# mttga/purejaxql

Hardware: NVIDIA H100
Metric: MinAtar-Breakout env steps/sec @4096 envs x128 seeds (higher is better)
Workload: dtype f32

## Files before the change

### purejaxql_b200/csrc/conv16.cuh

```cuda
#pragma once
#include <cuda_fp16.h>
#include <cuda_runtime.h>
#include <stdint.h>

#include "../../include/pqn_b200.h"
#include "tc_common.cuh"

namespace pqn {

constexpr float LN_EPS = 1e-6f;
constexpr int CONV_O = 16;
constexpr int CONV_PIX = 64;
constexpr int HID_CNN = 128;
constexpr int FLAT_CNN = CONV_PIX * CONV_O;

template <int C>
struct ConvCfg {
  static constexpr int TAPS = 9 * C;
  static constexpr int OBS_BITS = 100 * C;
  static constexpr int OBS_WORDS = (OBS_BITS + 31) / 32;
  static constexpr int PW = (OBS_WORDS + 3) / 4 * 4;
  static constexpr int SW = PW + 1;
};

template <int C>
struct PatchCfg {
  static constexpr int WORDS = (9 * C + 31) / 32;
};

template <int C>
__device__ __forceinline__ void patch_bits(const uint32_t* __restrict__ so, int pix, uint32_t (&w)[PatchCfg<C>::WORDS]) {
  constexpr int W = PatchCfg<C>::WORDS;
#pragma unroll
  for (int k = 0; k < W; ++k) w[k] = 0u;
  const int y = pix >> 3, x = pix & 7;
#pragma unroll
  for (int di = 0; di < 3; ++di) {
    const int f0 = ((y + di) * 10 + x) * C;
    const uint32_t r = __funnelshift_r(so[f0 >> 5], so[(f0 >> 5) + 1], f0 & 31) & ((1u << (3 * C)) - 1u);
    const int o = 3 * C * di;
    w[o >> 5] |= r << (o & 31);
    if ((o & 31) + 3 * C > 32) w[min((o >> 5) + 1, W - 1)] |= r >> (32 - (o & 31));
  }
}

__device__ __forceinline__ void ln16_quad(const float (&z)[2][4], float& mean0, float& rstd0, float& mean1,
                                          float& rstd1) {
  float s0 = z[0][0] + z[0][1] + z[1][0] + z[1][1];
  float q0 = fmaf(z[1][1], z[1][1], fmaf(z[1][0], z[1][0], fmaf(z[0][0], z[0][0], __fmul_rn(z[0][1], z[0][1]))));
  float s1 = z[0][2] + z[0][3] + z[1][2] + z[1][3];
  float q1 = fmaf(z[1][3], z[1][3], fmaf(z[1][2], z[1][2], fmaf(z[0][2], z[0][2], __fmul_rn(z[0][3], z[0][3]))));
#pragma unroll
  for (int o = 1; o <= 2; o <<= 1) {
    s0 += __shfl_xor_sync(0xffffffffu, s0, o); q0 += __shfl_xor_sync(0xffffffffu, q0, o);
    s1 += __shfl_xor_sync(0xffffffffu, s1, o); q1 += __shfl_xor_sync(0xffffffffu, q1, o);
  }
  mean0 = __fmul_rn(s0, 1.0f / CONV_O); mean1 = __fmul_rn(s1, 1.0f / CONV_O);
  rstd0 = rsqrtf(fmaxf(fmaf(q0, 1.0f / CONV_O, -__fmul_rn(mean0, mean0)), 0.f) + LN_EPS);
  rstd1 = rsqrtf(fmaxf(fmaf(q1, 1.0f / CONV_O, -__fmul_rn(mean1, mean1)), 0.f) + LN_EPS);
}

__device__ __forceinline__ void mma_f16_16n8k16(float (&d)[4], const uint32_t (&a)[4], uint32_t b0, uint32_t b1) {
  asm volatile(
      "mma.sync.aligned.m16n8k16.row.col.f32.f16.f16.f32 {%0,%1,%2,%3}, {%4,%5,%6,%7}, {%8,%9}, {%0,%1,%2,%3};"
      : "+f"(d[0]), "+f"(d[1]), "+f"(d[2]), "+f"(d[3])
      : "r"(a[0]), "r"(a[1]), "r"(a[2]), "r"(a[3]), "r"(b0), "r"(b1));
}

template <int C>
struct Conv16 {
  static constexpr int TAPS = 9 * C;
  static constexpr int KS = (TAPS + 15) / 16;
  static constexpr int ROW = 2 * KS < 8 ? 8 : 2 * KS;
};

__host__ __device__ constexpr int conv16_channel(int h, int n) { return 4 * (n >> 1) + 2 * h + (n & 1); }

__host__ __device__ constexpr int conv16_tap(int s, int kk) {
  return 16 * s + (kk < 8 ? 0 : 8) + ((kk & 1) ? 4 : 0) + ((kk & 7) >> 1);
}

template <int C>
__device__ __forceinline__ void conv16_load_weights(const float* __restrict__ prm, const pqn_net_layout_t& L, uint4* wb,
                                                    float* cb, float* sc, float* bi, int tid, int nt) {
  using M = Conv16<C>;
  const float inv255 = 1.0f / 255.0f;
  for (int i = tid; i < M::KS * 2 * 32; i += nt) {
    const int ln = i & 31, h = (i >> 5) & 1, s = i >> 6;
    const int gg = ln >> 2, tt = ln & 3;
    const int o = conv16_channel(h, gg);
    const float scale = __uint_as_float((uint32_t)(127 + 15 - (1 << tt)) << 23);
    float v[4];
#pragma unroll
    for (int q = 0; q < 4; ++q) {
      const int tap = conv16_tap(s, 2 * tt + (q & 1) + (q >> 1) * 8);
      v[q] = tap < M::TAPS ? __ldg(prm + L.conv_w + tap * CONV_O + o) * inv255 * scale : 0.f;
      v[q] = fminf(fmaxf(v[q], -65000.f), 65000.f);
    }
    const __half2 h0 = __floats2half2_rn(v[0], v[1]), h1 = __floats2half2_rn(v[2], v[3]);
    const float2 f0 = __half22float2(h0), f1 = __half22float2(h1);
    const __half2 l0 = __floats2half2_rn(v[0] - f0.x, v[1] - f0.y), l1 = __floats2half2_rn(v[2] - f1.x, v[3] - f1.y);
    wb[i] = make_uint4(*reinterpret_cast<const uint32_t*>(&h0), *reinterpret_cast<const uint32_t*>(&h1),
                       *reinterpret_cast<const uint32_t*>(&l0), *reinterpret_cast<const uint32_t*>(&l1));
  }
  if (tid < CONV_O) {
    cb[tid] = __ldg(prm + L.conv_b + tid);
    sc[tid] = __ldg(prm + L.ln0_scale + tid);
    bi[tid] = __ldg(prm + L.ln0_bias + tid);
  }
}

template <int C>
__device__ __forceinline__ void build_patch16(const uint32_t* __restrict__ so, int pix, uint32_t* __restrict__ out) {
  constexpr int W = PatchCfg<C>::WORDS;
  uint32_t w[W];
  patch_bits<C>(so, pix, w);
#pragma unroll
  for (int b = 0; b < 2 * Conv16<C>::KS; ++b) {
    const int o = 8 * b;
    uint32_t v = (o >> 5) < W ? w[(o >> 5) < W ? (o >> 5) : 0] : 0u;
    const int sh = o & 31;
    const uint32_t lo = sh >= 10 ? v >> (sh - 10) : v << (10 - sh);
    const uint32_t hi = sh + 4 <= 26 ? v << (26 - sh - 4) : v >> (sh + 4 - 26);
    out[b] = __byte_perm(lo, hi, 0x7610);
  }
}

template <int C>
__device__ __forceinline__ void store_patch16(const uint32_t* __restrict__ so, int pix, uint32_t* __restrict__ row) {
  using M = Conv16<C>;
  uint32_t w[M::ROW];
#pragma unroll
  for (int k = 0; k < M::ROW; ++k) w[k] = 0u;
  build_patch16<C>(so, pix, w);
#pragma unroll
  for (int q = 0; q < M::ROW / 4; ++q)
    *reinterpret_cast<uint4*>(row + 4 * q) = make_uint4(w[4 * q], w[4 * q + 1], w[4 * q + 2], w[4 * q + 3]);
}

template <int C, int NB>
__device__ __forceinline__ void conv16_blocks(const uint32_t* __restrict__ xp, const uint4* __restrict__ wb,
                                              const float* __restrict__ cb, int mb0, int lane, float (&z)[NB][2][4]) {
  using M = Conv16<C>;
  const int g = lane >> 2, t = lane & 3;
  const uint32_t mask = (1u << (10 + t)) | (1u << (26 + t));
#pragma unroll
  for (int i = 0; i < NB; ++i)
#pragma unroll
    for (int h = 0; h < 2; ++h) {
      z[i][h][0] = z[i][h][2] = cb[4 * t + 2 * h];
      z[i][h][1] = z[i][h][3] = cb[4 * t + 2 * h + 1];
    }
  const uint32_t* r00 = xp + (16 * mb0 + g) * M::ROW;
#pragma unroll
  for (int s = 0; s < M::KS; ++s) {
    uint32_t a[NB][4];
#pragma unroll
    for (int i = 0; i < NB; ++i) {
      const uint2 w0 = *reinterpret_cast<const uint2*>(r00 + (16 * i) * M::ROW + 2 * s);
      const uint2 w1 = *reinterpret_cast<const uint2*>(r00 + (16 * i + 8) * M::ROW + 2 * s);
      a[i][0] = w0.x & mask; a[i][1] = w1.x & mask; a[i][2] = w0.y & mask; a[i][3] = w1.y & mask;
    }
    uint4 b[2];
#pragma unroll
    for (int h = 0; h < 2; ++h) b[h] = wb[(s * 2 + h) * 32 + lane];
#pragma unroll
    for (int h = 0; h < 2; ++h)
#pragma unroll
      for (int i = 0; i < NB; ++i) mma_f16_16n8k16(z[i][h], a[i], b[h].z, b[h].w);
#pragma unroll
    for (int h = 0; h < 2; ++h)
#pragma unroll
      for (int i = 0; i < NB; ++i) mma_f16_16n8k16(z[i][h], a[i], b[h].x, b[h].y);
  }
}

__device__ __forceinline__ void conv16_xhat(const float (&z)[2][4], float (&x0)[4], float (&x1)[4], float& rstd0,
                                            float& rstd1) {
  float mean0, mean1;
  ln16_quad(z, mean0, rstd0, mean1, rstd1);
  const float nm0 = -__fmul_rn(mean0, rstd0), nm1 = -__fmul_rn(mean1, rstd1);
#pragma unroll
  for (int h = 0; h < 2; ++h)
#pragma unroll
    for (int c = 0; c < 2; ++c) {
      x0[2 * h + c] = fmaf(z[h][c], rstd0, nm0);
      x1[2 * h + c] = fmaf(z[h][2 + c], rstd1, nm1);
    }
}

__device__ __forceinline__ uint32_t cvt_f16x2_satfinite(float lo, float hi) {
  uint32_t r;
  asm("cvt.rn.satfinite.f16x2.f32 %0, %1, %2;" : "=r"(r) : "f"(hi), "f"(lo));
  return r;
}

__device__ __forceinline__ void conv16_act(const float (&z)[2][4], const float (&sc4)[4], const float (&bi4)[4],
                                           float (&v0)[4], float (&v1)[4]) {
  float x0[4], x1[4], rstd0, rstd1;
  conv16_xhat(z, x0, x1, rstd0, rstd1);
#pragma unroll
  for (int c = 0; c < 4; ++c) {
    v0[c] = fmaxf(fmaf(x0[c], sc4[c], bi4[c]), 0.f);
    v1[c] = fmaxf(fmaf(x1[c], sc4[c], bi4[c]), 0.f);
  }
}

__device__ __forceinline__ void conv16_split(const float (&v)[4], uint32_t (&hw)[2], uint32_t (&lw)[2]) {
#pragma unroll
  for (int h = 0; h < 2; ++h) {
    hw[h] = cvt_f16x2_satfinite(v[2 * h], v[2 * h + 1]);
    const float2 f = __half22float2(*reinterpret_cast<const __half2*>(&hw[h]));
    const __half2 l = __floats2half2_rn((v[2 * h] - f.x) * tc::TC_LO_SCALE, (v[2 * h + 1] - f.y) * tc::TC_LO_SCALE);
    lw[h] = *reinterpret_cast<const uint32_t*>(&l);
  }
}

namespace tc {
struct ConvIn {
  const uint32_t* obs;
  int64_t obs_rows_per_seed;
  const int32_t* gather;
  pqn_net_layout_t L;
};
int launch_conv_gemm16(int C, int epi, const CUtensorMap* tb, const GemmShape& gs, const EpiParams& ep, const ConvIn& ci,
                       cudaStream_t st, int kernel_id);
}


}
```

### purejaxql_b200/csrc/pqn_net.cu

```cuda
#include <cuda_runtime.h>
#include <stdint.h>

#include "../../include/pqn_b200.h"
#include "api_common.h"
#include "tc_common.cuh"
#include "conv16.cuh"

namespace pqn {

constexpr int GT = 256;
constexpr int BK = 16;

static int g_use_tc = 2;
static int g_conv_mma = 1;
static int g_conv_fuse = 1;

__host__ __device__ static inline int64_t align4(int64_t x) { return (x + 3) & ~(int64_t)3; }

static int make_layout(const pqn_net_desc_t* d, pqn_net_layout_t* L) {
  int64_t off = 0;
  auto take = [&](int64_t n) { int64_t o = off; off += align4(n); return o; };
  L->d1_w = L->d1_b = L->ln1_scale = L->ln1_bias = L->conv_w = L->conv_b = -1;
  L->gru_ir_w = L->gru_ir_b = L->gru_iz_w = L->gru_iz_b = L->gru_in_w = L->gru_in_b = -1;
  L->gru_hr_w = L->gru_hz_w = L->gru_hn_w = L->gru_hn_b = -1;
// ... 1388 lines not shown
  for (; row < rows; row += row_stride) {
    __syncwarp();
    if (lane < Cfg::PW) my_so[lane] = pre;
    if (lane == 0) my_so[Cfg::PW] = 0u;
    __syncwarp();
    pre = fetch_obs(row + row_stride);
    build_patches<C>(my_so, my_patch, lane);
    cp_async_wait_all();
    __syncwarp();
#pragma unroll 1
    for (int mb = 0; mb < 4; ++mb) {
      const int p0 = 16 * mb + g, p1 = p0 + 8;
      float z[2][4];
      float2 dyv[2][2];
#pragma unroll
      for (int h = 0; h < 2; ++h) {
        dyv[h][0] = *reinterpret_cast<const float2*>(my_dy + p0 * CONV_O + cswz(p0, 8 * h + 2 * t));
        dyv[h][1] = *reinterpret_cast<const float2*>(my_dy + p1 * CONV_O + cswz(p1, 8 * h + 2 * t));
        const float2 a0 = *reinterpret_cast<const float2*>(my_xh + p0 * CONV_O + cswz(p0, 8 * h + 2 * t));
        const float2 a1 = *reinterpret_cast<const float2*>(my_xh + p1 * CONV_O + cswz(p1, 8 * h + 2 * t));
        z[h][0] = a0.x; z[h][1] = a0.y; z[h][2] = a1.x; z[h][3] = a1.y;
      }
      const float rstd0 = my_rs[p0], rstd1 = my_rs[p1];
      float dxh[2][4];
      float m1a = 0.f, m2a = 0.f, m1b = 0.f, m2b = 0.f;
#pragma unroll
      for (int h = 0; h < 2; ++h) {
        const int o = 8 * h + 2 * t;
        const float dy4[4] = {dyv[h][0].x, dyv[h][0].y, dyv[h][1].x, dyv[h][1].y};
#pragma unroll
        for (int j = 0; j < 4; ++j) {
          const int col = 2 * h + (j & 1);
          a_dsc[col] = fmaf(dy4[j], z[h][j], a_dsc[col]);
          a_dbi[col] += dy4[j];
          dxh[h][j] = dy4[j] * sc[o + (j & 1)];
          if (j < 2) { m1a += dxh[h][j]; m2a = fmaf(dxh[h][j], z[h][j], m2a); }
          else { m1b += dxh[h][j]; m2b = fmaf(dxh[h][j], z[h][j], m2b); }
        }
      }
#pragma unroll
      for (int o = 1; o <= 2; o <<= 1) {
        m1a += __shfl_xor_sync(0xffffffffu, m1a, o); m2a += __shfl_xor_sync(0xffffffffu, m2a, o);
        m1b += __shfl_xor_sync(0xffffffffu, m1b, o); m2b += __shfl_xor_sync(0xffffffffu, m2b, o);
      }
      m1a *= (1.0f / CONV_O); m2a *= (1.0f / CONV_O); m1b *= (1.0f / CONV_O); m2b *= (1.0f / CONV_O);
#pragma unroll
      for (int h = 0; h < 2; ++h) {
        const int o = 8 * h + 2 * t;
        float dzv[4];
#pragma unroll
        for (int j = 0; j < 4; ++j) {
          const float rstd = j < 2 ? rstd0 : rstd1, m1 = j < 2 ? m1a : m1b, m2 = j < 2 ? m2a : m2b;
          dzv[j] = rstd * (dxh[h][j] - m1 - z[h][j] * m2);
          a_dcb[2 * h + (j & 1)] += dzv[j];
        }
        *reinterpret_cast<float2*>(my_dz + p0 * CDZ_LD + cswz(p0, o)) = make_float2(dzv[0], dzv[1]);
        *reinterpret_cast<float2*>(my_dz + p1 * CDZ_LD + cswz(p1, o)) = make_float2(dzv[2], dzv[3]);
      }
    }
    __syncwarp();
    fetch_rows(row + row_stride);
    float wacc[M::MT][2][4];
#pragma unroll
    for (int mt = 0; mt < M::MT; ++mt)
#pragma unroll
      for (int h = 0; h < 2; ++h)
#pragma unroll
        for (int j = 0; j < 4; ++j) wacc[mt][h][j] = 0.f;
#pragma unroll 1
    for (int kk = 0; kk < 8; ++kk) {
      uint32_t bh[2][2], bl[2][2];
#pragma unroll
      for (int h = 0; h < 2; ++h) {
        const int r0 = 8 * kk + t, r1 = r0 + 4;
        const float v0 = my_dz[r0 * CDZ_LD + cswz(r0, 8 * h + g)], v1 = my_dz[r1 * CDZ_LD + cswz(r1, 8 * h + g)];
        bh[h][0] = __float_as_uint(v0) & 0xFFFFE000u; bh[h][1] = __float_as_uint(v1) & 0xFFFFE000u;
        bl[h][0] = __float_as_uint(v0 - __uint_as_float(bh[h][0])); bl[h][1] = __float_as_uint(v1 - __uint_as_float(bh[h][1]));
      }
      const int pa = 8 * kk + t, pb = pa + 4;
      uint32_t qa[PWD], qb[PWD];
#pragma unroll
      for (int k = 0; k < PWD; ++k) { qa[k] = my_patch[pa * PWD + k]; qb[k] = my_patch[pb * PWD + k]; }
#pragma unroll
      for (int mt = 0; mt < M::MT; ++mt) {
        const uint32_t wa = qa[(16 * mt) >> 5], wb = qb[(16 * mt) >> 5];
        const int sh = ((16 * mt) & 31) + g;
        uint32_t a[4];
        a[0] = bit_f32(wa, sh); a[1] = bit_f32(wa, sh + 8); a[2] = bit_f32(wb, sh); a[3] = bit_f32(wb, sh + 8);
        if (__ballot_sync(0xffffffffu, (a[0] | a[1] | a[2] | a[3]) != 0u) == 0u) continue;
        mma_tf32_16n8k8(wacc[mt][0], a, bl[0][0], bl[0][1]);
        mma_tf32_16n8k8(wacc[mt][1], a, bl[1][0], bl[1][1]);
        mma_tf32_16n8k8(wacc[mt][0], a, bh[0][0], bh[0][1]);
        mma_tf32_16n8k8(wacc[mt][1], a, bh[1][0], bh[1][1]);
      }
    }
#pragma unroll
    for (int mt = 0; mt < M::MT; ++mt)
#pragma unroll
      for (int h = 0; h < 2; ++h)
#pragma unroll
        for (int j = 0; j < 4; ++j) wrun[mt][h][j] += wacc[mt][h][j];
  }
  cp_async_wait_all();
  __syncthreads();
  for (int w = 0; w < SM::WARPS; ++w) {
    if (warp == w) {
#pragma unroll
      for (int mt = 0; mt < M::MT; ++mt)
#pragma unroll
        for (int h = 0; h < 2; ++h)
#pragma unroll
          for (int j = 0; j < 4; ++j) {
            const int tap = 16 * mt + g + (j >= 2 ? 8 : 0);
            float* dst = &s_w[tap * CONV_O + 8 * h + 2 * t + (j & 1)];
            *dst = (w == 0 ? 0.f : *dst) + wrun[mt][h][j];
          }
    }
    __syncthreads();
  }
#pragma unroll
  for (int col = 0; col < 4; ++col) {
    float v0 = a_dsc[col], v1 = a_dbi[col], v2 = a_dcb[col];
#pragma unroll
    for (int sft = 4; sft <= 16; sft <<= 1) {
      v0 += __shfl_xor_sync(0xffffffffu, v0, sft);
      v1 += __shfl_xor_sync(0xffffffffu, v1, sft);
      v2 += __shfl_xor_sync(0xffffffffu, v2, sft);
    }
    a_dsc[col] = v0; a_dbi[col] = v1; a_dcb[col] = v2;
  }
  for (int w = 0; w < SM::WARPS; ++w) {
    if (warp == w && g == 0) {
#pragma unroll
      for (int col = 0; col < 4; ++col) {
        const int o = 8 * (col >> 1) + 2 * t + (col & 1);
        s_red[o] = (w == 0 ? 0.f : s_red[o]) + a_dsc[col];
        s_red[CONV_O + o] = (w == 0 ? 0.f : s_red[CONV_O + o]) + a_dbi[col];
        s_red[2 * CONV_O + o] = (w == 0 ? 0.f : s_red[2 * CONV_O + o]) + a_dcb[col];
      }
    }
    __syncthreads();
  }
  float* __restrict__ o = part + ((int64_t)seed * gridDim.x + blockIdx.x) * (M::TAPS * CONV_O + 3 * CONV_O);
  for (int i = tid; i < M::TAPS * CONV_O; i += blockDim.x) o[i] = s_w[i] * (1.0f / 255.0f);
  if (tid < 3 * CONV_O) o[M::TAPS * CONV_O + tid] = s_red[tid];
}

template <int C>
struct ConvBwd16 {
  static constexpr int MT = ConvMma<C>::MT;
  static constexpr int NG = 4 * MT;
  static constexpr int NGP = (NG % 8 == 4) ? NG : NG + 4;
  static constexpr int DY = 0;
  static constexpr int XH = DY + FLAT_CNN;
  static constexpr int RS = XH + 16 * CONV_O;
  static constexpr int DZT = RS + 16;
  static constexpr int PW = DZT + 2 * CONV_O * 32;
  static constexpr int XP = PW + 32 * NGP;
  static constexpr int WARP_FLOATS = (XP + CONV_PIX * Conv16<C>::ROW + 3) / 4 * 4;
  static constexpr int WARPS = (C == 4) ? 8 : 6;
  static constexpr int WB = WARPS * WARP_FLOATS;
  static constexpr int BYTES = (WB + Conv16<C>::KS * 2 * 32 * 4 + 6 * CONV_O) * 4;
};

__device__ __forceinline__ int cswz16(int p, int col) {
  return ((p ^ ((p >> 2) & 1)) << 4) + (col ^ (((p >> 1) & 1) << 3));
}
__device__ __forceinline__ int dzt_word(int ch, int ks, int pos) {
  const int c7 = ch & 7;
  return (ch << 5) + ((ks ^ ((c7 + (c7 >> 2)) & 3)) << 3) + pos;
}

template <int C>
__global__ void __launch_bounds__(ConvBwd16<C>::WARPS * 32, 2)
    conv_bwd_mma16_kernel(const uint32_t* __restrict__ obs, int64_t obs_rows_per_seed, const int32_t* __restrict__ gather,
                          const float* __restrict__ params, int64_t P, pqn_net_layout_t L, const float* __restrict__ DY1,
                          float* __restrict__ part, int rows, float gs) {
  using Cfg = ConvCfg<C>;
  using M = ConvMma<C>;
  using SM = ConvBwd16<C>;
  constexpr int PWD = PatchCfg<C>::WORDS;
  extern __shared__ __align__(16) float smem_bwd[];
  const int tid = threadIdx.x, warp = tid >> 5, lane = tid & 31;
  const int g = lane >> 2, t = lane & 3;
  const int seed = blockIdx.y;
  float* my = smem_bwd + warp * SM::WARP_FLOATS;
  float* my_dy = my + SM::DY;
  float* my_xh = my + SM::XH;
  float* my_rs = my + SM::RS;
  uint32_t* my_dzt = reinterpret_cast<uint32_t*>(my + SM::DZT);
  uint32_t* my_so = reinterpret_cast<uint32_t*>(my + SM::DZT);
  uint32_t* my_pw = reinterpret_cast<uint32_t*>(my + SM::PW);
  uint32_t* my_xp = reinterpret_cast<uint32_t*>(my + SM::XP);
  uint4* wb = reinterpret_cast<uint4*>(smem_bwd + SM::WB);
  float* cb = smem_bwd + SM::WB + Conv16<C>::KS * 2 * 32 * 4;
  float* sc = cb + CONV_O;
  float* bi = sc + CONV_O;
  float* s_red = bi + CONV_O;
  float* s_w = smem_bwd;
  static_assert(Cfg::SW <= 2 * CONV_O * 32, "obs staging aliases the dz planes");
  static_assert(M::MT * 16 * CONV_O <= SM::WARP_FLOATS * SM::WARPS, "dW reduction buffer aliases the warp slices");
  static_assert(Cfg::PW <= 32, "one packed observation word per lane");
  static_assert(SM::XP % 4 == 0 && SM::WB % 4 == 0, "16-byte aligned patch rows and weight fragments");
  conv16_load_weights<C>(params + (int64_t)seed * P, L, wb, cb, sc, bi, threadIdx.x, blockDim.x);
  if (tid < 3 * CONV_O) s_red[tid] = 0.f;
  __syncthreads();
  float a_dsc[4] = {0.f, 0.f, 0.f, 0.f}, a_dbi[4] = {0.f, 0.f, 0.f, 0.f}, a_dcb[4] = {0.f, 0.f, 0.f, 0.f};
  float wrun[M::MT][2][4];
#pragma unroll
  for (int mt = 0; mt < M::MT; ++mt)
#pragma unroll
    for (int h = 0; h < 2; ++h)
#pragma unroll
      for (int j = 0; j < 4; ++j) wrun[mt][h][j] = 0.f;
  const uint32_t amask = (1u << (10 + (g & 3))) | (1u << (26 + (g & 3)));
  const int pos_g = g < 4 ? 2 * g : 2 * (g - 4) + 1;

  const int row_stride = gridDim.x * SM::WARPS;
  auto fetch_index = [&](int r) -> int {
    const int rc = r < rows ? r : rows - 1;
    return gather ? __ldg(gather + (int64_t)seed * rows + rc) : rc;
  };
  auto fetch_obs = [&](int src) -> uint32_t {
    return __ldg(obs + ((int64_t)seed * obs_rows_per_seed + src) * Cfg::PW + (lane < Cfg::PW ? lane : 0));
  };
  auto fetch_dy = [&](int r) {
    if (r < rows) {
      const float* dsrc = DY1 + ((int64_t)seed * rows + r) * FLAT_CNN;
#pragma unroll
      for (int i = 0; i < FLAT_CNN / 4 / 32; ++i) {
        const int q = i * 32 + lane, prow = q >> 2;
        cp_async16(my_dy + cswz16(prow, (q & 3) * 4), dsrc + q * 4);
      }
    }
    cp_async_commit();
  };
  int row = blockIdx.x * SM::WARPS + warp;
  uint32_t pre = fetch_obs(fetch_index(row));
  int src_next = fetch_index(row + row_stride);
  fetch_dy(row);
  for (; row < rows; row += row_stride) {
    __syncwarp();
    if (lane < Cfg::PW) my_so[lane] = pre;
    if (lane == 0) my_so[Cfg::PW] = 0u;
    __syncwarp();
    pre = fetch_obs(src_next);
    src_next = fetch_index(row + 2 * row_stride);
    store_patch16<C>(my_so, lane, my_xp + lane * Conv16<C>::ROW);
    store_patch16<C>(my_so, lane + 32, my_xp + (lane + 32) * Conv16<C>::ROW);
    {
      uint32_t w0[PWD], w1[PWD];
      patch_bits<C>(my_so, 2 * lane, w0);
      patch_bits<C>(my_so, 2 * lane + 1, w1);
      uint32_t pw[SM::NGP];
#pragma unroll
      for (int k = 0; k < SM::NGP; ++k) pw[k] = 0u;
#pragma unroll
      for (int q = 0; q < SM::NG; ++q) {
        const int ql = q & 3, slot = (q & ~3) + (ql == 1 ? 2 : (ql == 2 ? 1 : ql));
        const int bit = 4 * q, wi = bit >> 5, sh = bit & 31;
        if (wi < PWD) {
          const uint32_t v0 = w0[wi < PWD ? wi : 0], v1 = w1[wi < PWD ? wi : 0];
          const uint32_t lo = sh >= 10 ? v0 >> (sh >= 10 ? sh - 10 : 0) : v0 << (sh < 10 ? 10 - sh : 0);
          const uint32_t hi = sh <= 26 ? v1 << (sh <= 26 ? 26 - sh : 0) : v1 >> (sh > 26 ? sh - 26 : 0);
          pw[slot] = __byte_perm(lo, hi, 0x7610);
        }
      }
      uint32_t* dstw = my_pw + lane * SM::NGP;
#pragma unroll
      for (int k = 0; k < SM::NGP / 4; ++k)
        *reinterpret_cast<uint4*>(dstw + 4 * k) = make_uint4(pw[4 * k], pw[4 * k + 1], pw[4 * k + 2], pw[4 * k + 3]);
    }
    cp_async_wait_all();
    __syncwarp();
#pragma unroll 1
    for (int mb = 0; mb < 4; ++mb) {
      {
        float zc[1][2][4], x0[4], x1[4], rs0, rs1;
        conv16_blocks<C, 1>(my_xp, wb, cb, mb, lane, zc);
        conv16_xhat(zc[0], x0, x1, rs0, rs1);
        __syncwarp();
        *reinterpret_cast<float4*>(my_xh + cswz16(g, 4 * t)) = make_float4(x0[0], x0[1], x0[2], x0[3]);
        *reinterpret_cast<float4*>(my_xh + cswz16(g + 8, 4 * t)) = make_float4(x1[0], x1[1], x1[2], x1[3]);
        if (t == 0) { my_rs[g] = rs0; my_rs[g + 8] = rs1; }
        __syncwarp();
      }
      const int p0 = 16 * mb + 2 * g, p1 = p0 + 1;
      float z[2][4];
      float2 dyv[2][2];
#pragma unroll
      for (int h = 0; h < 2; ++h) {
        dyv[h][0] = *reinterpret_cast<const float2*>(my_dy + cswz16(p0, 8 * h + 2 * t));
        dyv[h][1] = *reinterpret_cast<const float2*>(my_dy + cswz16(p1, 8 * h + 2 * t));
        const float2 a0 = *reinterpret_cast<const float2*>(my_xh + cswz16(2 * g, 8 * h + 2 * t));
        const float2 a1 = *reinterpret_cast<const float2*>(my_xh + cswz16(2 * g + 1, 8 * h + 2 * t));
        z[h][0] = a0.x; z[h][1] = a0.y; z[h][2] = a1.x; z[h][3] = a1.y;
      }
      const float rstd0 = my_rs[2 * g] * gs, rstd1 = my_rs[2 * g + 1] * gs;
      float dxh[2][4];
      float m1a = 0.f, m2a = 0.f, m1b = 0.f, m2b = 0.f;
#pragma unroll
      for (int h = 0; h < 2; ++h) {
        const int o = 8 * h + 2 * t;
        const float dy4[4] = {dyv[h][0].x, dyv[h][0].y, dyv[h][1].x, dyv[h][1].y};
#pragma unroll
        for (int j = 0; j < 4; ++j) {
          const int col = 2 * h + (j & 1);
          a_dsc[col] = fmaf(dy4[j], z[h][j], a_dsc[col]);
          a_dbi[col] += dy4[j];
          dxh[h][j] = dy4[j] * sc[o + (j & 1)];
          if (j < 2) { m1a += dxh[h][j]; m2a = fmaf(dxh[h][j], z[h][j], m2a); }
          else { m1b += dxh[h][j]; m2b = fmaf(dxh[h][j], z[h][j], m2b); }
        }
      }
#pragma unroll
      for (int o = 1; o <= 2; o <<= 1) {
        m1a += __shfl_xor_sync(0xffffffffu, m1a, o); m2a += __shfl_xor_sync(0xffffffffu, m2a, o);
        m1b += __shfl_xor_sync(0xffffffffu, m1b, o); m2b += __shfl_xor_sync(0xffffffffu, m2b, o);
      }
      m1a *= (1.0f / CONV_O); m2a *= (1.0f / CONV_O); m1b *= (1.0f / CONV_O); m2b *= (1.0f / CONV_O);
#pragma unroll
      for (int h = 0; h < 2; ++h) {
        float dzv[4];
#pragma unroll
        for (int j = 0; j < 4; ++j) {
          const float rstd = j < 2 ? rstd0 : rstd1, m1 = j < 2 ? m1a : m1b, m2 = j < 2 ? m2a : m2b;
          dzv[j] = rstd * (dxh[h][j] - m1 - z[h][j] * m2);
          a_dcb[2 * h + (j & 1)] += dzv[j];
        }
#pragma unroll
        for (int c = 0; c < 2; ++c) {
          const float v0 = dzv[c], v1 = dzv[2 + c];
          const uint32_t hw = cvt_f16x2_satfinite(v0, v1);
          const float2 hf = __half22float2(*reinterpret_cast<const __half2*>(&hw));
          const __half2 lw = __floats2half2_rn(v0 - hf.x, v1 - hf.y);
          const int wd = dzt_word(8 * h + 2 * t + c, mb, pos_g);
          my_dzt[wd] = hw;
          my_dzt[CONV_O * 32 + wd] = *reinterpret_cast<const uint32_t*>(&lw);
        }
      }
    }
    __syncwarp();
    fetch_dy(row + row_stride);
    float wacc[M::MT][2][4];
#pragma unroll
    for (int mt = 0; mt < M::MT; ++mt)
#pragma unroll
      for (int h = 0; h < 2; ++h)
#pragma unroll
        for (int j = 0; j < 4; ++j) wacc[mt][h][j] = 0.f;
#pragma unroll 1
    for (int ks = 0; ks < 4; ++ks) {
      uint2 bhi[2], blo[2];
#pragma unroll
      for (int h = 0; h < 2; ++h) {
        const int wd = dzt_word(8 * h + g, ks, 2 * t);
        bhi[h] = *reinterpret_cast<const uint2*>(my_dzt + wd);
        blo[h] = *reinterpret_cast<const uint2*>(my_dzt + CONV_O * 32 + wd);
      }
      const uint32_t* pa = my_pw + (8 * ks + t) * SM::NGP + 2 * (g >> 2);
      const uint32_t* pb = pa + 4 * SM::NGP;
#pragma unroll
      for (int mt = 0; mt < M::MT; ++mt) {
        const uint2 wa = *reinterpret_cast<const uint2*>(pa + 4 * mt), wb = *reinterpret_cast<const uint2*>(pb + 4 * mt);
        uint32_t a[4];
        a[0] = wa.x & amask; a[1] = wa.y & amask; a[2] = wb.x & amask; a[3] = wb.y & amask;
        mma_f16_16n8k16(wacc[mt][0], a, blo[0].x, blo[0].y);
        mma_f16_16n8k16(wacc[mt][1], a, blo[1].x, blo[1].y);
        mma_f16_16n8k16(wacc[mt][0], a, bhi[0].x, bhi[0].y);
        mma_f16_16n8k16(wacc[mt][1], a, bhi[1].x, bhi[1].y);
      }
    }
#pragma unroll
    for (int mt = 0; mt < M::MT; ++mt)
#pragma unroll
      for (int h = 0; h < 2; ++h)
#pragma unroll
        for (int j = 0; j < 4; ++j) wrun[mt][h][j] += wacc[mt][h][j];
  }
  cp_async_wait_all();
  const float inv_gs = 1.0f / gs;
  const float unscale = __uint_as_float((uint32_t)(127 + 15 - (1 << (g & 3))) << 23) * inv_gs;
  __syncthreads();
  for (int w = 0; w < SM::WARPS; ++w) {
    if (warp == w) {
#pragma unroll
      for (int mt = 0; mt < M::MT; ++mt)
#pragma unroll
        for (int h = 0; h < 2; ++h)
#pragma unroll
          for (int j = 0; j < 4; ++j) {
            const int tap = 16 * mt + g + (j >= 2 ? 8 : 0);
            float* dst = &s_w[tap * CONV_O + 8 * h + 2 * t + (j & 1)];
            *dst = (w == 0 ? 0.f : *dst) + wrun[mt][h][j] * unscale;
          }
    }
    __syncthreads();
  }
#pragma unroll
  for (int col = 0; col < 4; ++col) {
    float v0 = a_dsc[col], v1 = a_dbi[col], v2 = a_dcb[col];
#pragma unroll
    for (int sft = 4; sft <= 16; sft <<= 1) {
      v0 += __shfl_xor_sync(0xffffffffu, v0, sft);
      v1 += __shfl_xor_sync(0xffffffffu, v1, sft);
      v2 += __shfl_xor_sync(0xffffffffu, v2, sft);
    }
    a_dsc[col] = v0; a_dbi[col] = v1; a_dcb[col] = v2;
  }
  for (int w = 0; w < SM::WARPS; ++w) {
    if (warp == w && g == 0) {
#pragma unroll
      for (int col = 0; col < 4; ++col) {
        const int o = 8 * (col >> 1) + 2 * t + (col & 1);
        s_red[o] = (w == 0 ? 0.f : s_red[o]) + a_dsc[col];
        s_red[CONV_O + o] = (w == 0 ? 0.f : s_red[CONV_O + o]) + a_dbi[col];
        s_red[2 * CONV_O + o] = (w == 0 ? 0.f : s_red[2 * CONV_O + o]) + a_dcb[col] * inv_gs;
      }
    }
    __syncthreads();
  }
  float* __restrict__ o = part + ((int64_t)seed * gridDim.x + blockIdx.x) * (M::TAPS * CONV_O + 3 * CONV_O);
  for (int i = tid; i < M::TAPS * CONV_O; i += blockDim.x) o[i] = s_w[i] * (1.0f / 255.0f);
  if (tid < 3 * CONV_O) o[M::TAPS * CONV_O + tid] = s_red[tid];
}

template <int SL>
__global__ void conv_bwd_final_kernel(const float* __restrict__ part, int nctas, int taps16, float* __restrict__ grads,
                                      int64_t P, pqn_net_layout_t L) {
  const int seed = blockIdx.y;
  const int stride = taps16 + 3 * CONV_O;
  const int i = blockIdx.x * (256 / SL) + threadIdx.x % (256 / SL);
  const float v = ordered_partial_sum<SL>(part + (int64_t)seed * nctas * stride + i, nctas, stride, i < stride);
  if (i >= stride || threadIdx.x >= 256 / SL) return;
  float* __restrict__ gout = grads + (int64_t)seed * P;
  if (i < taps16) gout[L.conv_w + i] = v;
  else if (i < taps16 + CONV_O) gout[L.ln0_scale + (i - taps16)] = v;
  else if (i < taps16 + 2 * CONV_O) gout[L.ln0_bias + (i - taps16 - CONV_O)] = v;
  else gout[L.conv_b + (i - taps16 - 2 * CONV_O)] = v;
}

__global__ void gather_rows_kernel(const float* __restrict__ obs, int64_t obs_rows_per_seed,
                                   const int32_t* __restrict__ gather, float* __restrict__ out, int rows, int D) {
  const int seed = blockIdx.y;
  const int64_t g = (int64_t)blockIdx.x * blockDim.x + threadIdx.x;
  if (g >= (int64_t)rows * D) return;
  const int r = (int)(g / D), j = (int)(g - (int64_t)r * D);
  const int64_t src = gather ? gather[(int64_t)seed * rows + r] : r;
  const float v = __ldg(obs + ((int64_t)seed * obs_rows_per_seed + src) * D + j);
  out[((int64_t)seed * rows + r) * D + j] = v;
}

struct Workspace {
  float *h1, *h2, *xhat2, *rstd2, *dz2;
  float *h1_lo, *dz2_lo, *w1_lo;
  float *cxhat, *crstd;
  uint32_t* relu_bits;
  float *rb_part, *cb_part;
  float* wg_part;
  float *xg, *h[PQN_MAX_LAYERS], *xhat[PQN_MAX_LAYERS], *rstd[PQN_MAX_LAYERS], *dzl, *dh0;
  float *m16_h0, *m16_w, *m16_dz;
};

static int64_t wgrad_split_tiles() { return 4 * (int64_t)device_sm_count() + 16; }
static int wgrad_ksplit(int tiles_total, int k_blocks) {
  const int sms = device_sm_count();
  if (tiles_total >= sms) return 1;
  int ks = sms / tiles_total;
  if (ks > k_blocks / 8) ks = k_blocks / 8;
  if (ks < 1) ks = 1;
  while (ks > 1 && (int64_t)(ks - 1) * ((k_blocks + ks - 1) / ks) >= k_blocks) --ks;
  return ks;
}
template <int SL>
__global__ void wgrad_split_reduce_kernel(const float* __restrict__ part, int ksplit, int64_t split_stride, int64_t n_per_seed,
                                          float* __restrict__ out, int64_t out_seed_stride) {
  const int seed = blockIdx.y;
  const int64_t i = (int64_t)blockIdx.x * (256 / SL) + threadIdx.x % (256 / SL);
  const float v = ordered_partial_sum<SL>(part + (int64_t)seed * n_per_seed + i, ksplit, split_stride, i < n_per_seed);
  if (i < n_per_seed && threadIdx.x < 256 / SL) out[(int64_t)seed * out_seed_stride + i] = v;
}
static void launch_split_reduce(const float* part, int ksplit, int64_t split_stride, int64_t n, int S, float* out,
                                int64_t out_seed_stride, cudaStream_t st) {
  LaunchScope _ls(K_GRAD_FINAL, st);
  if (final_slices(ksplit) == 32)
    wgrad_split_reduce_kernel<32><<<dim3((unsigned)((n + 7) / 8), S), 256, 0, st>>>(part, ksplit, split_stride, n, out, out_seed_stride);
  else
    wgrad_split_reduce_kernel<8><<<dim3((unsigned)((n + 31) / 32), S), 256, 0, st>>>(part, ksplit, split_stride, n, out, out_seed_stride);
}

static inline int ffma_ntile(int N) { return N % 128 == 0 ? 128 : 64; }
static inline int ffma_tiles(int Kin, int N) { return (Kin + 127) / 128 * (N / ffma_ntile(N)); }

static void run_wgrad_ffma(const float* X, int64_t x_seed_stride, int ldx, const float* DZ, int64_t dz_seed_stride, int N,
                           float* grads, int64_t P, int64_t off_w, int rows, int Kin, int S, int splits, float* part,
                           cudaStream_t st) {
  { LaunchScope _ls(K_WGRAD, st);
    const dim3 grid((unsigned)((Kin + 127) / 128), (unsigned)(N / ffma_ntile(N)), (unsigned)(S * splits));
    if (ffma_ntile(N) == 128)
      wgrad_kernel<128><<<grid, GT, 0, st>>>(X, x_seed_stride, ldx, DZ, dz_seed_stride, N, grads, P, off_w, rows, Kin, splits, part);
    else
      wgrad_kernel<64><<<grid, GT, 0, st>>>(X, x_seed_stride, ldx, DZ, dz_seed_stride, N, grads, P, off_w, rows, Kin, splits, part); }
  if (splits > 1) {
    const int64_t n = (int64_t)Kin * N;
    launch_split_reduce(part, splits, (int64_t)S * n, n, S, grads + off_w, P, st);
  }
}

constexpr int THIN_KMAX = 8, THIN_ROWS = 128;
__global__ void __launch_bounds__(256) wgrad_thin_kernel(const float* __restrict__ X, int64_t x_seed_stride, int Kin,
                                                         const float* __restrict__ DZ, int64_t dz_seed_stride, int N,
                                                         float* __restrict__ part, int rows, int rows_per_chunk) {
  __shared__ float xs[THIN_ROWS * THIN_KMAX];
  __shared__ float4 red[256];
  const int seed = blockIdx.y, S = gridDim.y;
  const int cols4 = N >> 2;
  const int groups = 256 / cols4, c4 = threadIdx.x % cols4, grp = threadIdx.x / cols4;
  const float* __restrict__ Xs = X + (int64_t)seed * x_seed_stride;
  const float4* __restrict__ Zs = reinterpret_cast<const float4*>(DZ + (int64_t)seed * dz_seed_stride);
  const int r_begin = blockIdx.x * rows_per_chunk, r_end = min(rows, r_begin + rows_per_chunk);
  float4 acc[THIN_KMAX];
#pragma unroll
  for (int k = 0; k < THIN_KMAX; ++k) acc[k] = make_float4(0.f, 0.f, 0.f, 0.f);
  for (int r0 = r_begin; r0 < r_end; r0 += THIN_ROWS) {
    const int nr = min(THIN_ROWS, r_end - r0);
    __syncthreads();
    for (int i = threadIdx.x; i < nr * Kin; i += 256) {
      const int r = i / Kin, k = i - r * Kin;
      xs[r * THIN_KMAX + k] = __ldg(Xs + (int64_t)(r0 + r) * Kin + k);
    }
    __syncthreads();
#pragma unroll 4
    for (int r = grp; r < nr; r += groups) {
      const float4 z = __ldg(Zs + (int64_t)(r0 + r) * cols4 + c4);
#pragma unroll
      for (int k = 0; k < THIN_KMAX; ++k)
        if (k < Kin) {
          const float x = xs[r * THIN_KMAX + k];
          acc[k].x = fmaf(x, z.x, acc[k].x); acc[k].y = fmaf(x, z.y, acc[k].y);
          acc[k].z = fmaf(x, z.z, acc[k].z); acc[k].w = fmaf(x, z.w, acc[k].w);
        }
    }
  }
  float4* __restrict__ out = reinterpret_cast<float4*>(part + ((int64_t)blockIdx.x * S + seed) * Kin * N);
#pragma unroll
  for (int k = 0; k < THIN_KMAX; ++k) {
    if (k >= Kin) break;
    __syncthreads();
    red[threadIdx.x] = acc[k];
    __syncthreads();
    if (grp == 0) {
      float4 v = red[c4];
      for (int g = 1; g < groups; ++g) {
        const float4 o = red[g * cols4 + c4];
        v.x += o.x; v.y += o.y; v.z += o.z; v.w += o.w;
      }
      out[k * cols4 + c4] = v;
    }
  }
}

static int64_t part_ctas(int S) { return 6 * 4 * (int64_t)device_sm_count() + 2 * (int64_t)S; }
static int64_t row_bwd_part_floats(int N, int A);
static int wgrad_splits(int tiles, int S, int rows);
static inline unsigned cdiv(int64_t a, int64_t b) { return (unsigned)((a + b - 1) / b); }

static void run_wgrad_first(const float* X, const float* DZ, float* grads, int64_t P, int64_t off_w, int S, int rows,
                            int D, int H, float* part, float* wg_part, cudaStream_t st) {
  if (D <= THIN_KMAX) {
    int chunks = (2 * device_sm_count()) / S;
// ... 1052 lines not shown
```

Measured before the change: 36.34 million.

## Restructure conv backward to keep LN recompute in registers with paired patch rows

The conv backward kernel no longer stages normalized activations and rstd through shared memory. It recomputes the conv output per lane in a pixel-pair-interleaved layout that matches the dy fragments, so the LN backward runs directly in registers with quad shuffles. The patch rows are derived from the same bit-gather used for the dW operand instead of a separate store_patch16 pass. This shrinks the per-warp shared memory footprint, removes several syncwarps and smem round trips, and unrolls the dW k-loop, at the cost of more register pressure and a new swizzle scheme.

Result: faster. 37.46 million (median of 6 runs) (+3.1%).

```diff
diff --git a/purejaxql_b200/csrc/conv16.cuh b/purejaxql_b200/csrc/conv16.cuh
--- a/purejaxql_b200/csrc/conv16.cuh
+++ b/purejaxql_b200/csrc/conv16.cuh
@@ -138,41 +138,57 @@
     *reinterpret_cast<uint4*>(row + 4 * q) = make_uint4(w[4 * q], w[4 * q + 1], w[4 * q + 2], w[4 * q + 3]);
 }
 
+template <int C, int NB, int BSTRIDE, bool PAIRED = false>
+__device__ __forceinline__ void conv16_blocks_rows(const uint32_t* __restrict__ ra, const uint32_t* __restrict__ rb,
+                                                   const uint4* __restrict__ wb, const float (&cb4)[4], int lane,
+                                                   float (&z)[NB][2][4]) {
+  using M = Conv16<C>;
+  const int t = lane & 3;
+  const uint32_t mask = (1u << (10 + t)) | (1u << (26 + t));
+#pragma unroll
+  for (int i = 0; i < NB; ++i)
+#pragma unroll
+    for (int h = 0; h < 2; ++h) {
+      z[i][h][0] = z[i][h][2] = cb4[2 * h];
+      z[i][h][1] = z[i][h][3] = cb4[2 * h + 1];
+    }
+#pragma unroll
+  for (int s = 0; s < M::KS; ++s) {
+    uint32_t a[NB][4];
+#pragma unroll
+    for (int i = 0; i < NB; ++i) {
+      uint2 w0, w1;
+      if (PAIRED) {
+        const uint4 v = *reinterpret_cast<const uint4*>(ra + i * BSTRIDE + 4 * s);
+        w0 = make_uint2(v.x, v.y); w1 = make_uint2(v.z, v.w);
+      } else {
+        w0 = *reinterpret_cast<const uint2*>(ra + i * BSTRIDE + 2 * s);
+        w1 = *reinterpret_cast<const uint2*>(rb + i * BSTRIDE + 2 * s);
+      }
+      a[i][0] = w0.x & mask; a[i][1] = w1.x & mask; a[i][2] = w0.y & mask; a[i][3] = w1.y & mask;
+    }
+    uint4 b[2];
+#pragma unroll
+    for (int h = 0; h < 2; ++h) b[h] = wb[(s * 2 + h) * 32 + lane];
+#pragma unroll
+    for (int h = 0; h < 2; ++h)
+#pragma unroll
+      for (int i = 0; i < NB; ++i) mma_f16_16n8k16(z[i][h], a[i], b[h].z, b[h].w);
+#pragma unroll
+    for (int h = 0; h < 2; ++h)
+#pragma unroll
+      for (int i = 0; i < NB; ++i) mma_f16_16n8k16(z[i][h], a[i], b[h].x, b[h].y);
+  }
+}
+
 template <int C, int NB>
 __device__ __forceinline__ void conv16_blocks(const uint32_t* __restrict__ xp, const uint4* __restrict__ wb,
                                               const float* __restrict__ cb, int mb0, int lane, float (&z)[NB][2][4]) {
   using M = Conv16<C>;
   const int g = lane >> 2, t = lane & 3;
-  const uint32_t mask = (1u << (10 + t)) | (1u << (26 + t));
-#pragma unroll
-  for (int i = 0; i < NB; ++i)
-#pragma unroll
-    for (int h = 0; h < 2; ++h) {
-      z[i][h][0] = z[i][h][2] = cb[4 * t + 2 * h];
-      z[i][h][1] = z[i][h][3] = cb[4 * t + 2 * h + 1];
-    }
+  const float cb4[4] = {cb[4 * t], cb[4 * t + 1], cb[4 * t + 2], cb[4 * t + 3]};
   const uint32_t* r00 = xp + (16 * mb0 + g) * M::ROW;
-#pragma unroll
-  for (int s = 0; s < M::KS; ++s) {
-    uint32_t a[NB][4];
-#pragma unroll
-    for (int i = 0; i < NB; ++i) {
-      const uint2 w0 = *reinterpret_cast<const uint2*>(r00 + (16 * i) * M::ROW + 2 * s);
-      const uint2 w1 = *reinterpret_cast<const uint2*>(r00 + (16 * i + 8) * M::ROW + 2 * s);
-      a[i][0] = w0.x & mask; a[i][1] = w1.x & mask; a[i][2] = w0.y & mask; a[i][3] = w1.y & mask;
-    }
-    uint4 b[2];
-#pragma unroll
-    for (int h = 0; h < 2; ++h) b[h] = wb[(s * 2 + h) * 32 + lane];
-#pragma unroll
-    for (int h = 0; h < 2; ++h)
-#pragma unroll
-      for (int i = 0; i < NB; ++i) mma_f16_16n8k16(z[i][h], a[i], b[h].z, b[h].w);
-#pragma unroll
-    for (int h = 0; h < 2; ++h)
-#pragma unroll
-      for (int i = 0; i < NB; ++i) mma_f16_16n8k16(z[i][h], a[i], b[h].x, b[h].y);
-  }
+  conv16_blocks_rows<C, NB, 16 * M::ROW>(r00, r00 + 8 * M::ROW, wb, cb4, lane, z);
 }
 
 __device__ __forceinline__ void conv16_xhat(const float (&z)[2][4], float (&x0)[4], float (&x1)[4], float& rstd0,
diff --git a/purejaxql_b200/csrc/pqn_net.cu b/purejaxql_b200/csrc/pqn_net.cu
--- a/purejaxql_b200/csrc/pqn_net.cu
+++ b/purejaxql_b200/csrc/pqn_net.cu
@@ -1564,23 +1564,19 @@
   static constexpr int NG = 4 * MT;
   static constexpr int NGP = (NG % 8 == 4) ? NG : NG + 4;
   static constexpr int DY = 0;
-  static constexpr int XH = DY + FLAT_CNN;
-  static constexpr int RS = XH + 16 * CONV_O;
-  static constexpr int DZT = RS + 16;
+  static constexpr int DZT = DY + FLAT_CNN;
   static constexpr int PW = DZT + 2 * CONV_O * 32;
   static constexpr int XP = PW + 32 * NGP;
-  static constexpr int WARP_FLOATS = (XP + CONV_PIX * Conv16<C>::ROW + 3) / 4 * 4;
+  static constexpr int WARP_FLOATS = XP + 32 * NGP;
   static constexpr int WARPS = (C == 4) ? 8 : 6;
   static constexpr int WB = WARPS * WARP_FLOATS;
   static constexpr int BYTES = (WB + Conv16<C>::KS * 2 * 32 * 4 + 6 * CONV_O) * 4;
+  static constexpr int NBR = (C == 10) ? 1 : 2;
 };
 
-__device__ __forceinline__ int cswz16(int p, int col) {
-  return ((p ^ ((p >> 2) & 1)) << 4) + (col ^ (((p >> 1) & 1) << 3));
-}
+__device__ __forceinline__ int dy_off(int p, int q) { return ((p ^ ((p >> 1) & 1)) << 4) + 4 * q; }
 __device__ __forceinline__ int dzt_word(int ch, int ks, int pos) {
-  const int c7 = ch & 7;
-  return (ch << 5) + ((ks ^ ((c7 + (c7 >> 2)) & 3)) << 3) + pos;
+  return (ch << 5) + ((ks ^ (ch >> 2) ^ (ch & 3)) << 3) + pos;
 }
 
 template <int C>
@@ -1598,8 +1594,6 @@
   const int seed = blockIdx.y;
   float* my = smem_bwd + warp * SM::WARP_FLOATS;
   float* my_dy = my + SM::DY;
-  float* my_xh = my + SM::XH;
-  float* my_rs = my + SM::RS;
   uint32_t* my_dzt = reinterpret_cast<uint32_t*>(my + SM::DZT);
   uint32_t* my_so = reinterpret_cast<uint32_t*>(my + SM::DZT);
   uint32_t* my_pw = reinterpret_cast<uint32_t*>(my + SM::PW);
@@ -1614,6 +1608,7 @@
   static_assert(M::MT * 16 * CONV_O <= SM::WARP_FLOATS * SM::WARPS, "dW reduction buffer aliases the warp slices");
   static_assert(Cfg::PW <= 32, "one packed observation word per lane");
   static_assert(SM::XP % 4 == 0 && SM::WB % 4 == 0, "16-byte aligned patch rows and weight fragments");
+  static_assert(SM::NG == 4 * Conv16<C>::KS, "a pixel's patch words are exactly the pair words' tap groups");
   conv16_load_weights<C>(params + (int64_t)seed * P, L, wb, cb, sc, bi, threadIdx.x, blockDim.x);
   if (tid < 3 * CONV_O) s_red[tid] = 0.f;
   __syncthreads();
@@ -1627,6 +1622,12 @@
       for (int j = 0; j < 4; ++j) wrun[mt][h][j] = 0.f;
   const uint32_t amask = (1u << (10 + (g & 3))) | (1u << (26 + (g & 3)));
   const int pos_g = g < 4 ? 2 * g : 2 * (g - 4) + 1;
+  const uint32_t* xpg = my_xp + g * SM::NGP;
+  const float* dy0 = my_dy + dy_off(2 * g, t);
+  const float* dy1 = my_dy + dy_off(2 * g + 1, t);
+  const int dzs = dzt_word(4 * t, 0, pos_g), dzl = dzt_word(g, 0, 2 * t);
+  const uint32_t* pa = my_pw + t * SM::NGP + 2 * (g >> 2);
+  const uint32_t* pb = pa + 4 * SM::NGP;
 
   const int row_stride = gridDim.x * SM::WARPS;
   auto fetch_index = [&](int r) -> int {
@@ -1641,8 +1642,8 @@
       const float* dsrc = DY1 + ((int64_t)seed * rows + r) * FLAT_CNN;
 #pragma unroll
       for (int i = 0; i < FLAT_CNN / 4 / 32; ++i) {
-        const int q = i * 32 + lane, prow = q >> 2;
-        cp_async16(my_dy + cswz16(prow, (q & 3) * 4), dsrc + q * 4);
+        const int q = i * 32 + lane;
+        cp_async16(my_dy + dy_off(q >> 2, q & 3), dsrc + q * 4);
       }
     }
     cp_async_commit();
@@ -1658,95 +1659,105 @@
     __syncwarp();
     pre = fetch_obs(src_next);
     src_next = fetch_index(row + 2 * row_stride);
-    store_patch16<C>(my_so, lane, my_xp + lane * Conv16<C>::ROW);
-    store_patch16<C>(my_so, lane + 32, my_xp + (lane + 32) * Conv16<C>::ROW);
     {
       uint32_t w0[PWD], w1[PWD];
       patch_bits<C>(my_so, 2 * lane, w0);
       patch_bits<C>(my_so, 2 * lane + 1, w1);
-      uint32_t pw[SM::NGP];
-#pragma unroll
-      for (int k = 0; k < SM::NGP; ++k) pw[k] = 0u;
+      uint32_t gw[SM::NG];
 #pragma unroll
       for (int q = 0; q < SM::NG; ++q) {
-        const int ql = q & 3, slot = (q & ~3) + (ql == 1 ? 2 : (ql == 2 ? 1 : ql));
         const int bit = 4 * q, wi = bit >> 5, sh = bit & 31;
+        gw[q] = 0u;
         if (wi < PWD) {
           const uint32_t v0 = w0[wi < PWD ? wi : 0], v1 = w1[wi < PWD ? wi : 0];
           const uint32_t lo = sh >= 10 ? v0 >> (sh >= 10 ? sh - 10 : 0) : v0 << (sh < 10 ? 10 - sh : 0);
           const uint32_t hi = sh <= 26 ? v1 << (sh <= 26 ? 26 - sh : 0) : v1 >> (sh > 26 ? sh - 26 : 0);
-          pw[slot] = __byte_perm(lo, hi, 0x7610);
+          gw[q] = __byte_perm(lo, hi, 0x7610);
         }
+      }
+      uint32_t pw[SM::NGP];
+#pragma unroll
+      for (int k = 0; k < SM::NGP; ++k) pw[k] = 0u;
+#pragma unroll
+      for (int q = 0; q < SM::NG; ++q) {
+        const int ql = q & 3, slot = (q & ~3) + (ql == 1 ? 2 : (ql == 2 ? 1 : ql));
+        pw[slot] = gw[q];
       }
       uint32_t* dstw = my_pw + lane * SM::NGP;
 #pragma unroll
       for (int k = 0; k < SM::NGP / 4; ++k)
         *reinterpret_cast<uint4*>(dstw + 4 * k) = make_uint4(pw[4 * k], pw[4 * k + 1], pw[4 * k + 2], pw[4 * k + 3]);
+      uint32_t* dstx = my_xp + lane * SM::NGP;
+#pragma unroll
+      for (int s = 0; s < Conv16<C>::KS; ++s)
+        *reinterpret_cast<uint4*>(dstx + 4 * s) =
+            make_uint4(__byte_perm(gw[4 * s], gw[4 * s + 1], 0x5410), __byte_perm(gw[4 * s + 2], gw[4 * s + 3], 0x5410),
+                       __byte_perm(gw[4 * s], gw[4 * s + 1], 0x7632), __byte_perm(gw[4 * s + 2], gw[4 * s + 3], 0x7632));
     }
     cp_async_wait_all();
     __syncwarp();
 #pragma unroll 1
-    for (int mb = 0; mb < 4; ++mb) {
-      {
-        float zc[1][2][4], x0[4], x1[4], rs0, rs1;
-        conv16_blocks<C, 1>(my_xp, wb, cb, mb, lane, zc);
-        conv16_xhat(zc[0], x0, x1, rs0, rs1);
-        __syncwarp();
-        *reinterpret_cast<float4*>(my_xh + cswz16(g, 4 * t)) = make_float4(x0[0], x0[1], x0[2], x0[3]);
-        *reinterpret_cast<float4*>(my_xh + cswz16(g + 8, 4 * t)) = make_float4(x1[0], x1[1], x1[2], x1[3]);
-        if (t == 0) { my_rs[g] = rs0; my_rs[g + 8] = rs1; }
-        __syncwarp();
-      }
-      const int p0 = 16 * mb + 2 * g, p1 = p0 + 1;
-      float z[2][4];
-      float2 dyv[2][2];
-#pragma unroll
-      for (int h = 0; h < 2; ++h) {
-        dyv[h][0] = *reinterpret_cast<const float2*>(my_dy + cswz16(p0, 8 * h + 2 * t));
-        dyv[h][1] = *reinterpret_cast<const float2*>(my_dy + cswz16(p1, 8 * h + 2 * t));
-        const float2 a0 = *reinterpret_cast<const float2*>(my_xh + cswz16(2 * g, 8 * h + 2 * t));
-        const float2 a1 = *reinterpret_cast<const float2*>(my_xh + cswz16(2 * g + 1, 8 * h + 2 * t));
-        z[h][0] = a0.x; z[h][1] = a0.y; z[h][2] = a1.x; z[h][3] = a1.y;
-      }
-      const float rstd0 = my_rs[2 * g] * gs, rstd1 = my_rs[2 * g + 1] * gs;
-      float dxh[2][4];
-      float m1a = 0.f, m2a = 0.f, m1b = 0.f, m2b = 0.f;
-#pragma unroll
-      for (int h = 0; h < 2; ++h) {
-        const int o = 8 * h + 2 * t;
-        const float dy4[4] = {dyv[h][0].x, dyv[h][0].y, dyv[h][1].x, dyv[h][1].y};
-#pragma unroll
-        for (int j = 0; j < 4; ++j) {
-          const int col = 2 * h + (j & 1);
-          a_dsc[col] = fmaf(dy4[j], z[h][j], a_dsc[col]);
-          a_dbi[col] += dy4[j];
-          dxh[h][j] = dy4[j] * sc[o + (j & 1)];
-          if (j < 2) { m1a += dxh[h][j]; m2a = fmaf(dxh[h][j], z[h][j], m2a); }
-          else { m1b += dxh[h][j]; m2b = fmaf(dxh[h][j], z[h][j], m2b); }
+    for (int mp = 0; mp < 4 / SM::NBR; ++mp) {
+      float zc[SM::NBR][2][4];
+      const float4 cbv = *reinterpret_cast<const float4*>(cb + 4 * t);
+      const float cb4[4] = {cbv.x, cbv.y, cbv.z, cbv.w};
+      conv16_blocks_rows<C, SM::NBR, 8 * SM::NGP, true>(xpg + 8 * SM::NBR * mp * SM::NGP, nullptr, wb, cb4, lane, zc);
+#pragma unroll
+      for (int i = 0; i < SM::NBR; ++i) {
+        const int mb = SM::NBR * mp + i;
+        float x[2][4], rs[2];
+        conv16_xhat(zc[i], x[0], x[1], rs[0], rs[1]);
+        const float4 d0 = *reinterpret_cast<const float4*>(dy0 + 256 * mb);
+        const float4 d1 = *reinterpret_cast<const float4*>(dy1 + 256 * mb);
+        const float dy[2][4] = {{d0.x, d0.y, d0.z, d0.w}, {d1.x, d1.y, d1.z, d1.w}};
+        const float4 scv = *reinterpret_cast<const float4*>(sc + 4 * t);
+        const float sc4[4] = {scv.x, scv.y, scv.z, scv.w};
+        float dxh[2][4];
+#pragma unroll
+        for (int p = 0; p < 2; ++p)
+#pragma unroll
+          for (int k = 0; k < 4; ++k) {
+            a_dsc[k] = fmaf(dy[p][k], x[p][k], a_dsc[k]);
+            a_dbi[k] = __fadd_rn(a_dbi[k], dy[p][k]);
+            dxh[p][k] = __fmul_rn(dy[p][k], sc4[k]);
+          }
+        float m1[2], m2[2];
+#pragma unroll
+        for (int p = 0; p < 2; ++p) {
+          float s1[2], s2[2];
+#pragma unroll
+          for (int j = 0; j < 2; ++j) {
+            s1[j] = __fadd_rn(__fadd_rn(0.f, dxh[p][2 * j]), dxh[p][2 * j + 1]);
+            s2[j] = fmaf(dxh[p][2 * j + 1], x[p][2 * j + 1], fmaf(dxh[p][2 * j], x[p][2 * j], 0.f));
+          }
+#pragma unroll
+          for (int j = 0; j < 2; ++j) {
+            const float r1 = __shfl_xor_sync(0xffffffffu, s1[j], 2), r2 = __shfl_xor_sync(0xffffffffu, s2[j], 2);
+            s1[j] = __fadd_rn(__fadd_rn(r1, dxh[p][2 * j]), dxh[p][2 * j + 1]);
+            s2[j] = fmaf(dxh[p][2 * j + 1], x[p][2 * j + 1], fmaf(dxh[p][2 * j], x[p][2 * j], r2));
+          }
+          float q1 = __fadd_rn(s1[0], s1[1]), q2 = __fadd_rn(s2[0], s2[1]);
+          q1 = __fadd_rn(q1, __shfl_xor_sync(0xffffffffu, q1, 1));
+          q2 = __fadd_rn(q2, __shfl_xor_sync(0xffffffffu, q2, 1));
+          m1[p] = __shfl_sync(0xffffffffu, q1, lane | 2);
+          m2[p] = __fmul_rn(__shfl_sync(0xffffffffu, q2, lane | 2), 1.0f / CONV_O);
         }
-      }
-#pragma unroll
-      for (int o = 1; o <= 2; o <<= 1) {
-        m1a += __shfl_xor_sync(0xffffffffu, m1a, o); m2a += __shfl_xor_sync(0xffffffffu, m2a, o);
-        m1b += __shfl_xor_sync(0xffffffffu, m1b, o); m2b += __shfl_xor_sync(0xffffffffu, m2b, o);
-      }
-      m1a *= (1.0f / CONV_O); m2a *= (1.0f / CONV_O); m1b *= (1.0f / CONV_O); m2b *= (1.0f / CONV_O);
-#pragma unroll
-      for (int h = 0; h < 2; ++h) {
-        float dzv[4];
-#pragma unroll
-        for (int j = 0; j < 4; ++j) {
-          const float rstd = j < 2 ? rstd0 : rstd1, m1 = j < 2 ? m1a : m1b, m2 = j < 2 ? m2a : m2b;
-          dzv[j] = rstd * (dxh[h][j] - m1 - z[h][j] * m2);
-          a_dcb[2 * h + (j & 1)] += dzv[j];
+        float dz[2][4];
+#pragma unroll
+        for (int p = 0; p < 2; ++p) {
+          const float rsg = __fmul_rn(rs[p], gs);
+#pragma unroll
+          for (int k = 0; k < 4; ++k) {
+            dz[p][k] = __fmul_rn(rsg, fmaf(-x[p][k], m2[p], fmaf(m1[p], -1.0f / CONV_O, dxh[p][k])));
+            a_dcb[k] = __fadd_rn(a_dcb[k], dz[p][k]);
+          }
         }
 #pragma unroll
-        for (int c = 0; c < 2; ++c) {
-          const float v0 = dzv[c], v1 = dzv[2 + c];
-          const uint32_t hw = cvt_f16x2_satfinite(v0, v1);
+        for (int k = 0; k < 4; ++k) {
+          const uint32_t hw = cvt_f16x2_satfinite(dz[0][k], dz[1][k]);
           const float2 hf = __half22float2(*reinterpret_cast<const __half2*>(&hw));
-          const __half2 lw = __floats2half2_rn(v0 - hf.x, v1 - hf.y);
-          const int wd = dzt_word(8 * h + 2 * t + c, mb, pos_g);
+          const __half2 lw = __floats2half2_rn(dz[0][k] - hf.x, dz[1][k] - hf.y);
+          const int wd = (dzs ^ ((k ^ mb) << 3)) + 32 * k;
           my_dzt[wd] = hw;
           my_dzt[CONV_O * 32 + wd] = *reinterpret_cast<const uint32_t*>(&lw);
         }
@@ -1761,22 +1772,21 @@
       for (int h = 0; h < 2; ++h)
 #pragma unroll
         for (int j = 0; j < 4; ++j) wacc[mt][h][j] = 0.f;
-#pragma unroll 1
+#pragma unroll
     for (int ks = 0; ks < 4; ++ks) {
       uint2 bhi[2], blo[2];
 #pragma unroll
       for (int h = 0; h < 2; ++h) {
-        const int wd = dzt_word(8 * h + g, ks, 2 * t);
+        const int wd = (dzl ^ ((ks ^ 2 * h) << 3)) + 256 * h;
         bhi[h] = *reinterpret_cast<const uint2*>(my_dzt + wd);
         blo[h] = *reinterpret_cast<const uint2*>(my_dzt + CONV_O * 32 + wd);
       }
-      const uint32_t* pa = my_pw + (8 * ks + t) * SM::NGP + 2 * (g >> 2);
-      const uint32_t* pb = pa + 4 * SM::NGP;
 #pragma unroll
       for (int mt = 0; mt < M::MT; ++mt) {
-        const uint2 wa = *reinterpret_cast<const uint2*>(pa + 4 * mt), wb = *reinterpret_cast<const uint2*>(pb + 4 * mt);
+        const uint2 wa = *reinterpret_cast<const uint2*>(pa + 8 * ks * SM::NGP + 4 * mt);
+        const uint2 wb2 = *reinterpret_cast<const uint2*>(pb + 8 * ks * SM::NGP + 4 * mt);
         uint32_t a[4];
-        a[0] = wa.x & amask; a[1] = wa.y & amask; a[2] = wb.x & amask; a[3] = wb.y & amask;
+        a[0] = wa.x & amask; a[1] = wa.y & amask; a[2] = wb2.x & amask; a[3] = wb2.y & amask;
         mma_f16_16n8k16(wacc[mt][0], a, blo[0].x, blo[0].y);
         mma_f16_16n8k16(wacc[mt][1], a, blo[1].x, blo[1].y);
         mma_f16_16n8k16(wacc[mt][0], a, bhi[0].x, bhi[0].y);
@@ -1810,24 +1820,24 @@
     __syncthreads();
   }
 #pragma unroll
-  for (int col = 0; col < 4; ++col) {
-    float v0 = a_dsc[col], v1 = a_dbi[col], v2 = a_dcb[col];
+  for (int k = 0; k < 4; ++k) {
+    float v0 = a_dsc[k], v1 = a_dbi[k], v2 = a_dcb[k];
 #pragma unroll
     for (int sft = 4; sft <= 16; sft <<= 1) {
       v0 += __shfl_xor_sync(0xffffffffu, v0, sft);
       v1 += __shfl_xor_sync(0xffffffffu, v1, sft);
       v2 += __shfl_xor_sync(0xffffffffu, v2, sft);
     }
-    a_dsc[col] = v0; a_dbi[col] = v1; a_dcb[col] = v2;
+    a_dsc[k] = v0; a_dbi[k] = v1; a_dcb[k] = v2;
   }
   for (int w = 0; w < SM::WARPS; ++w) {
     if (warp == w && g == 0) {
 #pragma unroll
-      for (int col = 0; col < 4; ++col) {
-        const int o = 8 * (col >> 1) + 2 * t + (col & 1);
-        s_red[o] = (w == 0 ? 0.f : s_red[o]) + a_dsc[col];
-        s_red[CONV_O + o] = (w == 0 ? 0.f : s_red[CONV_O + o]) + a_dbi[col];
-        s_red[2 * CONV_O + o] = (w == 0 ? 0.f : s_red[2 * CONV_O + o]) + a_dcb[col] * inv_gs;
+      for (int k = 0; k < 4; ++k) {
+        const int o = 4 * t + k;
+        s_red[o] = (w == 0 ? 0.f : s_red[o]) + a_dsc[k];
+        s_red[CONV_O + o] = (w == 0 ? 0.f : s_red[CONV_O + o]) + a_dbi[k];
+        s_red[2 * CONV_O + o] = (w == 0 ? 0.f : s_red[2 * CONV_O + o]) + a_dcb[k] * inv_gs;
       }
     }
     __syncthreads();
```
